# MobilePerceptionLab/EventCalib

Measured on NVIDIA B200. Metric: events/sec (detection+residual eval), higher is better.
Workload: dtype int32 pixels / f64 fit + f64 residuals

## Files before the change

eventcalib_b200/csrc/ecb_api.cu:

```cuda
#include <sched.h>
#include <math.h>
#include <stdarg.h>
#include <stdio.h>
#include <string.h>

#include <algorithm>

#include "ecb_window.cuh"

int ecb_fail(ecb_ctx *ctx, int code, const char *fmt, ...) {
    char buf[512];
    va_list ap;
    va_start(ap, fmt);
    vsnprintf(buf, sizeof buf, fmt, ap);
    va_end(ap);
    if (ctx) ctx->err = buf;
    return code;
}

int ecb_check(ecb_ctx *ctx, cudaError_t e, const char *what) {
    if (e == cudaSuccess) return ECB_OK;
    return ecb_fail(ctx, ECB_ERR_CUDA, "CUDA error %s: %s", what, cudaGetErrorString(e));
}

// ... 102 lines not shown
        cudaGetLastError();
        return 0;
    }
    return n;
}

int ecb_ctx_create(int device, void *stream, ecb_ctx **out) {
    if (!out) return ECB_ERR_ARG;
    *out = nullptr;
    int count = 0;
    if (cudaGetDeviceCount(&count) != cudaSuccess || count <= 0 || device < 0 || device >= count) return ECB_ERR_CUDA;
    if (cudaSetDevice(device) != cudaSuccess) return ECB_ERR_CUDA;
    ecb_ctx *c = new ecb_ctx();
    c->device = device;
    cudaDeviceProp prop;
    if (cudaGetDeviceProperties(&prop, device) != cudaSuccess) {
        delete c;
        return ECB_ERR_CUDA;
    }
    c->sm_count = prop.multiProcessorCount;
    c->smem_optin = (int) prop.sharedMemPerBlockOptin;
    if (stream) {
        c->stream = (cudaStream_t) stream;
    } else {
        if (cudaStreamCreateWithFlags(&c->stream, cudaStreamNonBlocking) != cudaSuccess) {
            delete c;
            return ECB_ERR_CUDA;
        }
        c->own_stream = true;
    }
    if (const char *e = getenv("ECB_BLOCKING_SYNC"))
        if (atoi(e) > 0 && cudaEventCreateWithFlags(&c->sync_ev, (atoi(e) == 1 ? cudaEventBlockingSync : 0) | cudaEventDisableTiming) == cudaSuccess)
            c->sync_mode = atoi(e) == 1 ? 1 : 2;
    *out = c;
    return ECB_OK;
}

void ecb_cost_free(ecb_ctx *ctx);
void ecb_covariance_free(ecb_ctx *ctx);

void ecb_ctx_destroy(ecb_ctx *c) {
    if (!c) return;
    cudaSetDevice(c->device);
    cudaStreamSynchronize(c->stream);
    ecb_covariance_free(c);
    ecb_cost_free(c);
    DevBuf *bufs[] = {&c->ev_raw, &c->ev_t, &c->ev_xyp, &c->ev_flag, &c->win_t, &c->win_lohi, &c->win_ptoff, &c->summary,
                      &c->arrive, &c->pts[0], &c->pts[1], &c->labels[0], &c->labels[1], &c->scratch, &c->ktab, &c->kmem,
                      &c->cand, &c->status, &c->db_pix, &c->db_off, &c->db_labels, &c->db_hdr, &c->db_scratch, &c->db_dims,
                      &c->fit_in, &c->fit_off, &c->fit_out, &c->db_hdr_b, &c->db_ktab, &c->db_counter, &c->kd_tree, &c->bfs_key,
                      &c->bfs_items, &c->bfs_front, &c->bfs_tab, &c->ord_htab, &c->pair_tab, &c->pose_io};
    for (DevBuf *b : bufs)
        if (b->p) cudaFree(b->p);
    for (DevBuf &b : c->gh)
        if (b.p) cudaFree(b.p);
    for (int i = 0; i < ECB_N_STAGES; ++i)
        for (int j = 0; j < 2; ++j)
            if (c->pev[i][j]) cudaEventDestroy(c->pev[i][j]);
    if (c->sync_ev) cudaEventDestroy(c->sync_ev);
    if (c->pinned) cudaFreeHost(c->pinned);
    if (c->up) cudaFreeHost(c->up);
    if (c->own_stream) cudaStreamDestroy(c->stream);
    delete c;
}

const char *ecb_last_error(const ecb_ctx *ctx) { return ctx ? ctx->err.c_str() : "null context"; }
// ... 655 lines not shown
```

eventcalib_b200/csrc/ecb_common.cuh:

```cuda
#pragma once
#include <cuda_runtime.h>
#include <stdint.h>

#include <string>
#include <vector>

#include "../../include/eventcalib_b200.h"

#define ECB_MAX_EPS 15
#define ECB_NONE 0xFFFFFFFFu
#define ECB_GH_MAXD 4
#define ECB_GH_NBUF 32

#define ECB_PIX_X(p) ((p) & 0x7FFFu)
#define ECB_PIX_Y(p) (((p) >> 15) & 0x7FFFu)
#define ECB_PIX_POL(p) ((p) >> 31)
#define ECB_PIX_XY(p) ((p) & 0x3FFFFFFFu)
#define ECB_PIX_INVALID 0x40000000u

struct DevBuf {
    void *p = nullptr;
    size_t cap = 0;
};

struct ecb_ctx {
    int device = 0;
    cudaStream_t stream = nullptr;
    bool own_stream = false;
    std::string err;
    uint64_t launches = 0;
    int sm_count = 148;
    int smem_optin = 0;
    int width = 0, height = 0;
    bool prof = false;
    int sync_mode = 0;
    cudaEvent_t sync_ev = nullptr;
    cudaEvent_t pev[ECB_N_STAGES][2] = {};
    bool pev_used[ECB_N_STAGES] = {};

    int64_t n_events = 0;
    DevBuf ev_raw, ev_t, ev_xyp, ev_flag;
    int n_win = 0;
    ecb_frontend_params fp{};
    DevBuf win_t, win_lohi, win_ptoff, summary, arrive, pts[2], labels[2], scratch, ktab, kmem, cand, status, pair_tab;
    int max_k_auto = 128;
    std::vector<int64_t> h_lohi, h_ptoff;
    int64_t total_points = 0;
    int cand_stride = 0;
    DevBuf kd_tree, bfs_key, bfs_items, bfs_front, bfs_tab;
    DevBuf ord_htab;
    int ord_htab_n = 0;
    DevBuf db_pix, db_off, db_labels, db_hdr, db_scratch, db_dims, db_hdr_b, db_ktab, db_counter;
    DevBuf gh[ECB_GH_NBUF];
    DevBuf fit_in, fit_off, fit_out;
    void *pinned = nullptr;
    size_t pinned_cap = 0;
    void *up = nullptr;
    size_t up_cap = 0, up_off = 0;
    void *cost = nullptr;
    void *cov = nullptr;
    uint64_t spline_gen = 0;
    uint32_t const_intrinsics = 0;
    DevBuf pose_io;
    uint64_t events_gen = 0;
};

struct EcbSplineView {
    const double *knots;
// ... 40 lines not shown
__device__ __forceinline__ uint32_t warp_incl_scan(uint32_t v) {
    const unsigned lane = threadIdx.x & 31;
#pragma unroll
    for (int o = 1; o < 32; o <<= 1) {
        uint32_t t = __shfl_up_sync(0xffffffffu, v, o);
        if (lane >= (unsigned) o) v += t;
    }
    return v;
}

__device__ __forceinline__ uint32_t block_excl_scan(uint32_t v, uint32_t *ws, uint32_t *total) {
    const unsigned lane = threadIdx.x & 31, wid = threadIdx.x >> 5, nw = (blockDim.x + 31) >> 5;
    uint32_t inc = warp_incl_scan(v);
    __syncthreads();
    if (lane == 31) ws[wid] = inc;
    __syncthreads();
    if (wid == 0) {
        uint32_t w = lane < nw ? ws[lane] : 0;
        uint32_t wi = warp_incl_scan(w);
        ws[lane] = wi - w;
        if (lane == 31) ws[32] = wi;
    }
    __syncthreads();
    *total = ws[32];
    return ws[wid] + inc - v;
}

__device__ __forceinline__ uint32_t row_bits(const uint32_t *row, int x0, int len) {
    const int wi = x0 >> 5, sh = x0 & 31;
    uint64_t v = (uint64_t) row[wi] | ((uint64_t) row[wi + 1] << 32);
    return (uint32_t) (v >> sh) & (len >= 32 ? 0xFFFFFFFFu : ((1u << len) - 1u));
}
__device__ __forceinline__ uint32_t test_bit(const uint32_t *row, int x) { return (row[x >> 5] >> (x & 31)) & 1u; }
#endif
```

eventcalib_b200/csrc/ecb_cost.cu:

```cuda
#include <stdlib.h>
#include <string.h>

#include <algorithm>
#include <cmath>
#include <vector>

#include "ecb_bspline.cuh"
#include "ecb_camera.h"
#include "ecb_common.cuh"
#include "ecb_residual_so3.h"

namespace {

constexpr int NE_THREADS = 256;
constexpr int NE_WARPS = NE_THREADS / 32;
constexpr int TILE_ROWS = 34, TILE_LD = 36;
constexpr int N_TILES = 10;
constexpr int PART_E32 = N_TILES * 64, PART_E33 = PART_E32 + 32, PART_SC = PART_E33 + 32, PART_STRIDE = PART_SC + 8;
constexpr int CHUNK = 2048;
constexpr int OUT_STRIDE = 33 * 33 + 33;

struct CostState {
    int n_splines = 0, total_cp = 0, total_spans = 0;
    std::vector<int> n_cp, cp_off, span_off, knot_off;
    std::vector<double> knots;
    double radius = 1.75, huber = 0.35;
    bool use_circ = false;
    int so3 = 0;
    int64_t n_res = 0;
    int n_items = 0;
    DevBuf d_knots, d_knot_off, d_ncp, d_cp_off, d_span_off;
    DevBuf obs, lm, tt, spl, basis, cp0, span;
    DevBuf span_start, items, part, out, params, cost_part, flags;
    DevBuf ev_flag, ev_cnt, ev_tag, kf_t, kf_circ, kf_c32, lm_tab, sel_event, sel_circle;
    std::vector<int64_t> h_span_start;
    bool assoc = false;
    int assoc_K = 0, assoc_n_circ = 0;
    uint64_t assoc_events_gen = 0;
    const double *assoc_kf_t = nullptr;
    double assoc_gate2 = 0.0;
    DevBuf rep_r, rep_key[2], rep_idx[2], rep_hist, rep_start, rep_out, rep_kf;
    DevBuf rep_io;
    DevBuf rej[9];
    uint64_t xch_last_epoch = 0;
    uint32_t xch_generation = 0;
};

CostState *state(ecb_ctx *ctx) {
    if (!ctx->cost) ctx->cost = new CostState();
    return (CostState *) ctx->cost;
}

__global__ void k_prepare(const double *__restrict__ t, const int *__restrict__ spl, int64_t n, const double *__restrict__ knots,
                          const int *__restrict__ knot_off, const int *__restrict__ ncp, const int *__restrict__ cp_off,
                          const int *__restrict__ span_off, double *__restrict__ basis, int *__restrict__ cp0,
                          int *__restrict__ span, uint32_t *__restrict__ flags) {
    const int64_t k = (int64_t) blockIdx.x * blockDim.x + threadIdx.x;
    if (k >= n) return;
    const int s = spl[k];
    const double *kn = knots + knot_off[s];
    const int nk = ncp[s] + 4;
    const double u = t[k];
    if (!(u >= kn[0] && u <= kn[nk - 1])) {
        atomicOr(flags, 1u);
        span[k] = 0;
        cp0[k] = 0;
        return;
// ... 17 lines not shown
    int64_t lo = 0, hi = n;
    while (lo < hi) {
        int64_t m = (lo + hi) >> 1;
        if (span[m] < s) lo = m + 1; else hi = m;
    }
    start[s] = lo;
}

struct Item {
    int64_t begin, end;
    int span, pad;
};

struct NeArgs {
    const double *obs, *lm, *basis;
    const int *circ;
    const double *lm_tab;
    const int *cp0;
    const Item *items;
    int n_items;
    const double *params;
    int total_cp;
    double radius, huber;
    double *part;
    const int *go;
};

__device__ __forceinline__ void dmma(double &c0, double &c1, double a, double b) {
    asm volatile("mma.sync.aligned.m8n8k4.row.col.f64.f64.f64.f64 {%0,%1}, {%2}, {%3}, {%0,%1};\n"
                 : "+d"(c0), "+d"(c1)
                 : "d"(a), "d"(b));
}

template <int MINB, bool SO3>
__global__ void __launch_bounds__(NE_THREADS, MINB) k_normal_eq(const NeArgs a) {
    extern __shared__ __align__(16) double sm_tiles[];
    if (a.go && *a.go == 0) return;
    const int lane = threadIdx.x & 31, wid = threadIdx.x >> 5;
    double *tile = sm_tiles + (size_t) wid * TILE_ROWS * TILE_LD;
    const int g = lane >> 2, t = lane & 3;
    const double *intr = a.params, *rot = a.params + 9, *trans = a.params + 9 + 4 * (size_t) a.total_cp;
    const int gw = blockIdx.x * NE_WARPS + wid, nw = gridDim.x * NE_WARPS;
    for (int it = gw; it < a.n_items; it += nw) {
        const Item item = a.items[it];
        double acc[N_TILES][2];
#pragma unroll
        for (int i = 0; i < N_TILES; ++i) acc[i][0] = acc[i][1] = 0.0;
        double e32 = 0.0, e33 = 0.0;
        double s3232 = 0.0, s3233 = 0.0, s3333 = 0.0, cost = 0.0;
        for (int64_t base = item.begin; base < item.end; base += 32) {
            const int64_t k = base + lane;
            double res = 0.0;
            __syncwarp();
            if (k < item.end) {
                const int c0 = a.cp0[k];
                const double4 b4 = reinterpret_cast<const double4 *>(a.basis)[k];
                const double b[4] = {b4.x, b4.y, b4.z, b4.w};
                const double2 o = reinterpret_cast<const double2 *>(a.obs)[k];
                const double *L = a.circ ? a.lm_tab + 3 * a.circ[k] : a.lm + 3 * k;
                const double Lx = L[0], Ly = L[1], Lz = L[2];
                const EcbResidualOut r =
                    SO3 ? ecb_residual_so3<true, TILE_LD>(intr, rot + 4 * (size_t) c0, trans + 3 * (size_t) c0, b, o.x, o.y,
                                                          Lx, Ly, Lz, a.radius, a.huber,
                                                          tile + lane)
                        : ecb_residual<true, TILE_LD>(intr, rot + 4 * (size_t) c0, trans + 3 * (size_t) c0, b, o.x, o.y,
                                                      Lx, Ly, Lz, a.radius, a.huber,
                                                      tile + lane);
                res = r.res;
                cost += r.cost;
            } else {
#pragma unroll
                for (int c = 0; c < 33; ++c) tile[c * TILE_LD + lane] = 0.0;
            }
            tile[33 * TILE_LD + lane] = res;
            __syncwarp();
            {
                const double x32 = tile[32 * TILE_LD + lane];
                s3232 += x32 * x32;
                s3233 += x32 * res;
                s3333 += res * res;
            }
#pragma unroll
            for (int ks = 0; ks < 8; ++ks) {
                double f[4];
#pragma unroll
                for (int G = 0; G < 4; ++G) f[G] = tile[(8 * G + g) * TILE_LD + 4 * ks + t];
                int ti = 0;
#pragma unroll
                for (int I = 0; I < 4; ++I)
#pragma unroll
                    for (int Jt = I; Jt < 4; ++Jt) {
                        dmma(acc[ti][0], acc[ti][1], f[I], f[Jt]);
                        ++ti;
                    }
#pragma unroll
                for (int q = 0; q < 4; ++q) {
                    const int kk = (4 * ks + q + (lane >> 2)) & 31;
                    const double aj = tile[lane * TILE_LD + kk];
                    e32 += aj * tile[32 * TILE_LD + kk];
                    e33 += aj * tile[33 * TILE_LD + kk];
                }
            }
        }
        double *p = a.part + (size_t) it * PART_STRIDE;
#pragma unroll
        for (int ti = 0; ti < N_TILES; ++ti) reinterpret_cast<double2 *>(p + ti * 64)[lane] = make_double2(acc[ti][0], acc[ti][1]);
        p[PART_E32 + lane] = e32;
        p[PART_E33 + lane] = e33;
#pragma unroll
        for (int o = 16; o > 0; o >>= 1) {
            cost += __shfl_xor_sync(0xffffffffu, cost, o);
            s3232 += __shfl_xor_sync(0xffffffffu, s3232, o);
            s3233 += __shfl_xor_sync(0xffffffffu, s3233, o);
            s3333 += __shfl_xor_sync(0xffffffffu, s3333, o);
        }
        if (lane == 0) {
            p[PART_SC + 0] = s3232;
            p[PART_SC + 1] = s3233;
            p[PART_SC + 2] = s3333;
            p[PART_SC + 3] = cost;
        }
    }
}

__global__ void k_reduce_spans(const double *__restrict__ part, const int *__restrict__ item_start, int n_spans,
                               double *__restrict__ out, const int *__restrict__ go = nullptr) {
    const int s = blockIdx.x;
    if (s >= n_spans || (go && *go == 0)) return;
    const int i0 = item_start[s], i1 = item_start[s + 1];
    double *o = out + (size_t) s * OUT_STRIDE;
    for (int e = threadIdx.x; e < PART_SC + 2; e += blockDim.x) {
        double v = 0.0;
        for (int it = i0; it < i1; ++it) v += part[(size_t) it * PART_STRIDE + e];
        if (e < PART_E32) {
            const int ti = e >> 6, r = (e >> 3) & 7, c = e & 7;
            int I = 0, rem = ti;
            while (rem >= 4 - I) {
                rem -= 4 - I;
                ++I;
            }
            const int Jt = I + rem;
            const int i = 8 * I + r, j = 8 * Jt + c;
            if (I != Jt || i <= j) {
                o[i * 33 + j] = v;
                o[j * 33 + i] = v;
            }
        } else if (e < PART_E33) {
            const int j = e - PART_E32;
            o[32 * 33 + j] = v;
            o[j * 33 + 32] = v;
        } else if (e < PART_SC) {
            o[1089 + (e - PART_E33)] = v;
        } else if (e == PART_SC) {
// ... 177 lines not shown
    const double *intr = params, *rot = params + 9, *trans = params + 9 + 4 * (size_t) total_cp;
    double c = 0.0;
    for (int64_t k = (int64_t) blockIdx.x * 256 + threadIdx.x; k < n; k += (int64_t) gridDim.x * 256) {
        const int c0 = cp0[k];
        const double4 b4 = reinterpret_cast<const double4 *>(basis)[k];
        const double b[4] = {b4.x, b4.y, b4.z, b4.w};
        const double2 o = reinterpret_cast<const double2 *>(obs)[k];
        const double *L = circ ? lm_tab + 3 * circ[k] : lm + 3 * k;
        const double Lx = L[0], Ly = L[1], Lz = L[2];
        c += SO3 ? ecb_residual_so3<false>(intr, rot + 4 * (size_t) c0, trans + 3 * (size_t) c0, b, o.x, o.y, Lx, Ly, Lz, radius,
                                           huber, nullptr).cost
                 : ecb_residual<false>(intr, rot + 4 * (size_t) c0, trans + 3 * (size_t) c0, b, o.x, o.y, Lx, Ly, Lz, radius, huber,
                                       nullptr).cost;
    }
    sh[threadIdx.x] = c;
    __syncthreads();
    for (int o = 128; o > 0; o >>= 1) {
        if (threadIdx.x < o) sh[threadIdx.x] += sh[threadIdx.x + o];
        __syncthreads();
    }
    if (threadIdx.x == 0) block_part[blockIdx.x] = sh[0];
}

struct AssocArgs {
    const double *ev_t;
    const uint32_t *ev_xyp;
    int64_t n_ev;
    const double *knots;
    const int *knot_off, *ncp;
    int n_splines;
    const double *kf_t, *kf_circ, *lm_tab;
    const float2 *kf_c32;
    int K, n_circ, n_circ32;
    double gate2;
    const int *cp_off, *span_off;
    double *basis;
    int *cp0, *span;
};

__device__ __forceinline__ int segment_of(const AssocArgs &a, double u) {
    for (int q = 0; q < a.n_splines; ++q) {
        const double *kn = a.knots + a.knot_off[q];
        if (u >= kn[0] && u <= kn[a.ncp[q] + 3]) return q;
    }
    return -1;
}

__device__ __forceinline__ int assoc_one(const AssocArgs &a, int64_t i, int *spline_out) {
    const double u = a.ev_t[i];
    const int s = segment_of(a, u);
    if (s < 0) return -1;
    *spline_out = s;
    int lo = 0, hi = a.K;
    while (lo < hi) {
        const int m = (lo + hi) >> 1;
        if (a.kf_t[m] < u) lo = m + 1; else hi = m;
    }
    int best = lo < a.K ? lo : a.K - 1;
    if (lo > 0 && (lo >= a.K || (u - a.kf_t[lo - 1]) <= (a.kf_t[lo] - u))) best = lo - 1;
    const double dt = u - a.kf_t[best];
    if (!(__dmul_rn(dt, dt) < a.gate2)) return -1;
    const uint32_t e = a.ev_xyp[i];
    if (e & ECB_PIX_INVALID) return -1;
    const double x = (double) ECB_PIX_X(e), y = (double) ECB_PIX_Y(e);
    const double *c = a.kf_circ + (size_t) best * a.n_circ * 3;
    int bi = -1;
    double bd = 0.0;
    {
        const float xf = (float) ECB_PIX_X(e), yf = (float) ECB_PIX_Y(e);
        const float4 *c4 = reinterpret_cast<const float4 *>(a.kf_c32 + (size_t) best * a.n_circ32);
        uint32_t k1 = 0xFFFFFFFFu, k2 = 0xFFFFFFFFu;
#pragma unroll 6
        for (int q = 0; q < a.n_circ32; q += 2) {
            const float4 cc = c4[q >> 1];
            const float dx0 = xf - cc.x, dy0 = yf - cc.y, dx1 = xf - cc.z, dy1 = yf - cc.w;
            const uint32_t ka = (__float_as_uint(fmaf(dx0, dx0, dy0 * dy0)) & 0xFFFFFF00u) | (uint32_t) q;
            const uint32_t kb = (__float_as_uint(fmaf(dx1, dx1, dy1 * dy1)) & 0xFFFFFF00u) | (uint32_t) (q + 1);
            k2 = min(k2, max(ka, k1));
            k1 = min(k1, ka);
            k2 = min(k2, max(kb, k1));
            k1 = min(k1, kb);
        }
        const float d1 = __uint_as_float(k1 & 0xFFFFFF00u), d2 = __uint_as_float(k2 | 0xFFu);
        if (d2 > d1 * 1.0001f + 0.02f) {
            bi = (int) (k1 & 0xFFu);
            if (bi >= a.n_circ || c[3 * bi + 2] < 0) return -1;
            const double dx = x - c[3 * bi], dy = y - c[3 * bi + 1];
            bd = __dadd_rn(__dmul_rn(dx, dx), __dmul_rn(dy, dy));
        } else {
            for (int q = 0; q < a.n_circ; ++q) {
                if (c[3 * q + 2] < 0) continue;
                const double dx = x - c[3 * q], dy = y - c[3 * q + 1];
                const double dd = __dadd_rn(__dmul_rn(dx, dx), __dmul_rn(dy, dy));
                if (bi < 0 || dd < bd) {
                    bi = q;
                    bd = dd;
                }
            }
        }
    }
    if (bi < 0) return -1;
    if (!(fabs(sqrt(bd) - c[3 * bi + 2]) < 5.0)) return -1;
    return bi;
}

constexpr int AS_THREADS = 256;

__global__ void k_circ32(const double *__restrict__ c, int K, int n_circ, int n_circ32, float2 *__restrict__ o) {
    const int i = blockIdx.x * blockDim.x + threadIdx.x;
    if (i >= K * n_circ32) return;
    const int k = i / n_circ32, q = i - k * n_circ32;
    float2 v = make_float2(3e18f, 3e18f);
    if (q < n_circ) {
        const double *p = c + ((size_t) k * n_circ + q) * 3;
        if (!(p[2] < 0)) v = make_float2((float) p[0], (float) p[1]);
    }
    o[i] = v;
}

__device__ __forceinline__ int nearest_kf(const double *kf_t, int K, double u) {
    int lo = 0, hi = K;
    while (lo < hi) {
        const int m = (lo + hi) >> 1;
        if (kf_t[m] < u) lo = m + 1; else hi = m;
    }
    int best = lo < K ? lo : K - 1;
    if (lo > 0 && (lo >= K || (u - kf_t[lo - 1]) <= (kf_t[lo] - u))) best = lo - 1;
    return best;
}

__global__ void __launch_bounds__(AS_THREADS) k_assoc_count(const AssocArgs a, uint16_t *__restrict__ tag,
                                                           uint32_t *__restrict__ block_cnt) {
    __shared__ uint32_t ws[33];
    const int64_t i = (int64_t) blockIdx.x * AS_THREADS + threadIdx.x;
    int s = 0;
    const int bi = i < a.n_ev ? assoc_one(a, i, &s) : -1;
    if (i < a.n_ev) tag[i] = bi >= 0 ? (uint16_t) ((s << 8) | (bi + 1)) : (uint16_t) 0;
    uint32_t tot;
    block_excl_scan(bi >= 0 ? 1u : 0u, ws, &tot);
    if (threadIdx.x == 0) block_cnt[blockIdx.x] = tot;
}

__global__ void k_scan_blocks(uint32_t *cnt, int n, int64_t *off, int64_t *total) {
    __shared__ uint32_t ws[33];
    const int per = (n + (int) blockDim.x - 1) / (int) blockDim.x;
    const int b = min(n, (int) threadIdx.x * per), e = min(n, b + per);
    uint32_t sum = 0;
    for (int i = b; i < e; ++i) sum += cnt[i];
    uint32_t tot;
    int64_t run = block_excl_scan(sum, ws, &tot);
    for (int i = b; i < e; ++i) {
        off[i] = run;
        run += cnt[i];
    }
    if (threadIdx.x == 0) *total = tot;
}

__global__ void __launch_bounds__(AS_THREADS) k_assoc_write(const AssocArgs a, const uint16_t *__restrict__ tag,
                                                           const int64_t *__restrict__ block_off,
                                                           double *__restrict__ obs, double *__restrict__ lm,
                                                           double *__restrict__ tt, int *__restrict__ spl,
                                                           int64_t *__restrict__ sel_event, int *__restrict__ sel_circle) {
    __shared__ uint32_t ws[33];
    const int64_t i = (int64_t) blockIdx.x * AS_THREADS + threadIdx.x;
    const uint32_t tg = i < a.n_ev ? tag[i] : 0u;
    uint32_t tot;
    const uint32_t ex = block_excl_scan(tg ? 1u : 0u, ws, &tot);
    if (tg) {
        const int bi = (int) (tg & 0xFF) - 1, s = (int) (tg >> 8);
// ... 712 lines not shown
    int rc;
    const int64_t n = ctx->n_events;
    const int nb = (int) ((n + AS_THREADS - 1) / AS_THREADS);
    if (!on_device) {
        if ((rc = ecb_reserve(ctx, st->kf_t, (size_t) n_keyframes * 8))) return rc;
        if ((rc = ecb_reserve(ctx, st->kf_circ, (size_t) n_keyframes * n_circles * 24))) return rc;
    }
    if ((rc = ecb_reserve(ctx, st->lm_tab, (size_t) n_circles * 24))) return rc;
    const int n_circ32 = (n_circles + 1) & ~1;
    if ((rc = ecb_reserve(ctx, st->kf_c32, (size_t) n_keyframes * n_circ32 * 8))) return rc;
    if (n_circles > 254 || st->n_splines > 255) return ecb_fail(ctx, ECB_ERR_UNSUPPORTED, "more than 254 circles or 255 spline segments");
    if ((rc = ecb_reserve(ctx, st->ev_cnt, (size_t) nb * 4 + 16))) return rc;
    if ((rc = ecb_reserve(ctx, st->ev_tag, (size_t) n * 2 + 16))) return rc;
    if ((rc = ecb_reserve(ctx, st->ev_flag, (size_t) nb * 8 + 16))) return rc;
    const double *d_kf_t = kf_time, *d_kf_circ = kf_circles;
    if (!on_device) {
        if ((rc = ecb_h2d(ctx, st->kf_t.p, kf_time, (size_t) n_keyframes * 8))) return rc;
        if ((rc = ecb_h2d(ctx, st->kf_circ.p, kf_circles, (size_t) n_keyframes * n_circles * 24))) return rc;
        if ((rc = ecb_h2d(ctx, st->lm_tab.p, landmarks_xyz, (size_t) n_circles * 24))) return rc;
        d_kf_t = (const double *) st->kf_t.p;
        d_kf_circ = (const double *) st->kf_circ.p;
    } else {
        ECB_CUDA(ctx, cudaMemcpyAsync(st->lm_tab.p, landmarks_xyz, (size_t) n_circles * 24, cudaMemcpyDeviceToDevice, ctx->stream));
    }
    AssocArgs a;
    assoc_args(ctx, st, a);
    a.kf_t = d_kf_t;
    a.kf_circ = d_kf_circ;
    a.kf_c32 = (const float2 *) st->kf_c32.p;
    a.K = n_keyframes;
    a.n_circ = n_circles;
    a.n_circ32 = n_circ32;
    a.gate2 = 5 * motion_time_step * 5 * motion_time_step;
    ECB_PROF_BEGIN(ctx, ECB_STAGE_ASSOC);
    k_circ32<<<(n_keyframes * n_circ32 + 255) / 256, 256, 0, ctx->stream>>>(d_kf_circ, n_keyframes, n_circles,
                                                                           n_circ32, (float2 *) st->kf_c32.p);
    ECB_LAUNCHED(ctx);
    k_assoc_count<<<nb, AS_THREADS, 0, ctx->stream>>>(a, (uint16_t *) st->ev_tag.p, (uint32_t *) st->ev_cnt.p);
    ECB_LAUNCHED(ctx);
    int64_t *d_total = (int64_t *) st->ev_flag.p + nb;
    k_scan_blocks<<<1, 1024, 0, ctx->stream>>>((uint32_t *) st->ev_cnt.p, nb, (int64_t *) st->ev_flag.p, d_total);
    ECB_LAUNCHED(ctx);
    int64_t total = 0;
    if ((rc = ecb_d2h(ctx, &total, d_total, 8))) return rc;
    bool fused = true;
    {
        std::vector<std::pair<double, double>> rg;
        size_t ko2 = 0;
        for (int q = 0; q < st->n_splines; ++q) {
            rg.emplace_back(st->knots[ko2], st->knots[ko2 + (size_t) st->n_cp[(size_t) q] + 3]);
            ko2 += (size_t) st->n_cp[(size_t) q] + 4;
        }
        std::sort(rg.begin(), rg.end());
        for (size_t q = 1; q < rg.size(); ++q)
            if (!(rg[q].first > rg[q - 1].second))
                return ecb_fail(ctx, ECB_ERR_UNSUPPORTED,
                                "spline knot ranges overlap ([%g, %g] and [%g, %g]): an event inside both would need one residual "
                                "per spline", rg[q - 1].first, rg[q - 1].second, rg[q].first, rg[q].second);
        size_t ko = 0;
        double prev_end = -1e300;
        for (int q = 0; q < st->n_splines; ++q) {
            const double b = st->knots[ko], e = st->knots[ko + (size_t) st->n_cp[(size_t) q] + 3];
            if (!(b > prev_end)) fused = false;
            prev_end = e;
            ko += (size_t) st->n_cp[(size_t) q] + 4;
        }
    }
    if ((rc = write_assoc_records(ctx, st, a, nb, total, fused))) return rc;
    ECB_PROF_END(ctx, ECB_STAGE_ASSOC);
    if ((rc = ecb_check(ctx, cudaGetLastError(), "association kernels"))) return rc;
    st->n_res = total;
// ... 24 lines not shown

static long long exchange_timeout_clocks(ecb_ctx *ctx) {
    static const double secs = getenv("ECB_EXCHANGE_TIMEOUT_S") ? atof(getenv("ECB_EXCHANGE_TIMEOUT_S")) : 30.0;
    static int khz_of[64] = {0};
    const int d = ctx->device & 63;
    if (khz_of[d] == 0) {
        int khz = 1965000;
        cudaDeviceGetAttribute(&khz, cudaDevAttrClockRate, ctx->device);
        khz_of[d] = khz > 0 ? khz : 1965000;
    }
    return (long long) (secs * 1e3 * (double) khz_of[d]);
}

static void fill_ne_args(CostState *st, NeArgs &a, const double *d_params, const int *d_go) {
    a.obs = (const double *) st->obs.p;
    a.lm = (const double *) st->lm.p;
    a.circ = st->use_circ ? (const int *) st->sel_circle.p : nullptr;
    a.lm_tab = (const double *) st->lm_tab.p;
    a.basis = (const double *) st->basis.p;
    a.cp0 = (const int *) st->cp0.p;
    a.items = (const Item *) st->items.p;
    a.n_items = st->n_items;
    a.params = d_params;
    a.total_cp = st->total_cp;
    a.radius = st->radius;
    a.huber = st->huber;
    a.part = (double *) st->part.p;
    a.go = d_go;
}

static int launch_normal_eq_kernel(ecb_ctx *ctx, CostState *st, const double *d_params, const int *d_go) {
    NeArgs a;
    fill_ne_args(st, a, d_params, d_go);
    const size_t smem = (size_t) NE_WARPS * TILE_ROWS * TILE_LD * 8;
    static const int variant = getenv("ECB_NE_VARIANT") ? atoi(getenv("ECB_NE_VARIANT")) : 2;
    void (*kern)(const NeArgs) = st->so3 ? k_normal_eq<1, true> : (variant == 1 ? k_normal_eq<1, false> : k_normal_eq<2, false>);
    ECB_CUDA(ctx, cudaFuncSetAttribute(kern, cudaFuncAttributeMaxDynamicSharedMemorySize, (int) smem));
    const int grid = std::min((st->n_items + NE_WARPS - 1) / NE_WARPS, ctx->sm_count * ((variant == 1 || st->so3) ? 1 : 2));
    kern<<<grid, NE_THREADS, smem, ctx->stream>>>(a);
    ECB_LAUNCHED(ctx);
    return ECB_OK;
}

static const int *item_start_of(CostState *st) {
    return (const int *) ((const char *) st->items.p + (size_t) std::max(st->n_items, 1) * sizeof(Item));
}

static void span_range(CostState *st, int &lo, int &hi) {
    lo = 0;
    hi = -1;
    for (int s = 0; s < st->total_spans; ++s)
        if (st->h_span_start[(size_t) s + 1] > st->h_span_start[(size_t) s]) {
            if (hi < 0) lo = s;
            hi = s;
        }
}

int ecb_cost_dev_eval(ecb_ctx *ctx, const double *d_params, const int *d_go, double *d_cost) {
    CostState *st = (CostState *) ctx->cost;
    int rc;
    if ((rc = ecb_reserve(ctx, st->cost_part, 4096 * 8))) return rc;
    if (st->n_res == 0) {
        ECB_CUDA(ctx, cudaMemsetAsync(d_cost, 0, 8, ctx->stream));
        return ECB_OK;
    }
    const int grid = (int) std::min<int64_t>((st->n_res + 255) / 256, (int64_t) ctx->sm_count * 8);
// ... 619 lines not shown
```

eventcalib_b200/csrc/ecb_window.cu:

```cuda
#include "ecb_cluster.cuh"
#include "ecb_window.cuh"

namespace {

constexpr int ING_REC = 256;
constexpr int ING_BYTES = ING_REC * 25;
constexpr int ING_THREADS = 256;

__device__ __forceinline__ uint32_t ld_unaligned32(const uint32_t *w, int byte_off) {
    const int wi = byte_off >> 2, sh = (byte_off & 3) * 8;
    return __funnelshift_r(w[wi], w[wi + 1], sh);
}

constexpr int ING_STAGES = 4;

__device__ __forceinline__ uint32_t smem_u32(const void *p) { return (uint32_t) __cvta_generic_to_shared(p); }
__device__ __forceinline__ void mbar_init(uint64_t *bar, int count) {
    asm volatile("mbarrier.init.shared::cta.b64 [%0], %1;" ::"r"(smem_u32(bar)), "r"(count));
}
__device__ __forceinline__ void mbar_expect_tx(uint64_t *bar, uint32_t bytes) {
    asm volatile("mbarrier.arrive.expect_tx.shared::cta.b64 _, [%0], %1;" ::"r"(smem_u32(bar)), "r"(bytes) : "memory");
}
__device__ __forceinline__ void mbar_wait(uint64_t *bar, uint32_t parity) {
    asm volatile(
        "{\n"
        ".reg .pred p;\n"
        "WAIT_%=:\n"
        "mbarrier.try_wait.parity.shared::cta.b64 p, [%0], %1;\n"
        "@p bra DONE_%=;\n"
        "bra WAIT_%=;\n"
        "DONE_%=:\n"
        "}" ::"r"(smem_u32(bar)), "r"(parity) : "memory");
}
__device__ __forceinline__ void bulk_g2s(void *dst, const void *src, uint32_t bytes, uint64_t *bar) {
    asm volatile("cp.async.bulk.shared::cluster.global.mbarrier::complete_tx::bytes [%0], [%1], %2, [%3];" ::"r"(smem_u32(dst)),
                 "l"(src), "r"(bytes), "r"(smem_u32(bar))
                 : "memory");
}

__global__ void __launch_bounds__(ING_THREADS) k_ingest(const uint8_t *__restrict__ raw, int64_t n, int W, int H,
                                                         double *__restrict__ out_t, uint32_t *__restrict__ out_xyp,
                                                         uint32_t *__restrict__ flags) {
    __shared__ __align__(128) uint32_t sm[ING_STAGES][ING_BYTES / 4 + 4];
    __shared__ __align__(8) uint64_t full[ING_STAGES];
    const int64_t n_tiles = (n + ING_REC - 1) / ING_REC;
    const int64_t total_bytes = n * 25;
    const int tid = threadIdx.x;
    const int64_t my_tiles = n_tiles > blockIdx.x ? (n_tiles - blockIdx.x + gridDim.x - 1) / gridDim.x : 0;
    auto issue = [&](int64_t it) {
        const int st = (int) (it % ING_STAGES);
        const int64_t byte0 = (blockIdx.x + it * gridDim.x) * (int64_t) ING_BYTES;
        const uint32_t bytes = (uint32_t) (min((int64_t) ING_BYTES, total_bytes - byte0) & ~(int64_t) 15);
        mbar_expect_tx(&full[st], bytes);
        if (bytes) bulk_g2s(sm[st], raw + byte0, bytes, &full[st]);
    };
    if (tid == 0) {
        for (int st = 0; st < ING_STAGES; ++st) mbar_init(&full[st], 1);
        asm volatile("fence.mbarrier_init.release.cluster;" ::: "memory");
    }
    __syncthreads();
    if (tid == 0)
        for (int64_t it = 0; it < my_tiles && it < ING_STAGES; ++it) issue(it);
    uint32_t bad = 0;
    for (int64_t it = 0; it < my_tiles; ++it) {
        const int st = (int) (it % ING_STAGES);
// ... 239 lines not shown
```

Measured before the change: 2.619 billion.

## Add per-keyframe spatial cell candidate lists for event-circle association

Builds a per-keyframe grid of 16x16 pixel cells, each holding up to 7 candidate circles that could be nearest to any pixel in the cell. The association kernel then checks only those candidates and falls back to the full scan when a cell overflows or the nearest two are too close to call. The aim is to replace the full scan over all circles per event with a few lookups. It costs an extra precompute kernel with a shared array of fixed size (254 circles), and it adds a risk of results differing when the candidate bounds are near ties.

```diff
diff --git a/eventcalib_b200/csrc/ecb_api.cu b/eventcalib_b200/csrc/ecb_api.cu
--- a/eventcalib_b200/csrc/ecb_api.cu
+++ b/eventcalib_b200/csrc/ecb_api.cu
@@ -158,6 +158,7 @@
     if (const char *e = getenv("ECB_BLOCKING_SYNC"))
         if (atoi(e) > 0 && cudaEventCreateWithFlags(&c->sync_ev, (atoi(e) == 1 ? cudaEventBlockingSync : 0) | cudaEventDisableTiming) == cudaSuccess)
             c->sync_mode = atoi(e) == 1 ? 1 : 2;
+    if (const char *e = getenv("ECB_ASSOC_SCAN")) c->assoc_scan = atoi(e) == 1;
     *out = c;
     return ECB_OK;
 }
diff --git a/eventcalib_b200/csrc/ecb_common.cuh b/eventcalib_b200/csrc/ecb_common.cuh
--- a/eventcalib_b200/csrc/ecb_common.cuh
+++ b/eventcalib_b200/csrc/ecb_common.cuh
@@ -34,6 +34,7 @@
     int width = 0, height = 0;
     bool prof = false;
     int sync_mode = 0;
+    bool assoc_scan = false;
     cudaEvent_t sync_ev = nullptr;
     cudaEvent_t pev[ECB_N_STAGES][2] = {};
     bool pev_used[ECB_N_STAGES] = {};
diff --git a/eventcalib_b200/csrc/ecb_cost.cu b/eventcalib_b200/csrc/ecb_cost.cu
--- a/eventcalib_b200/csrc/ecb_cost.cu
+++ b/eventcalib_b200/csrc/ecb_cost.cu
@@ -32,7 +32,7 @@
     DevBuf d_knots, d_knot_off, d_ncp, d_cp_off, d_span_off;
     DevBuf obs, lm, tt, spl, basis, cp0, span;
     DevBuf span_start, items, part, out, params, cost_part, flags;
-    DevBuf ev_flag, ev_cnt, ev_tag, kf_t, kf_circ, kf_c32, lm_tab, sel_event, sel_circle;
+    DevBuf ev_flag, ev_cnt, ev_tag, kf_t, kf_circ, kf_c32, kf_cells, lm_tab, sel_event, sel_circle;
     std::vector<int64_t> h_span_start;
     bool assoc = false;
     int assoc_K = 0, assoc_n_circ = 0;
@@ -446,6 +446,8 @@
     const double *kf_t, *kf_circ, *lm_tab;
     const float2 *kf_c32;
     int K, n_circ, n_circ32;
+    const uint2 *cells;
+    int cell_nx, cell_ny;
     double gate2;
     const int *cp_off, *span_off;
     double *basis;
@@ -460,26 +462,22 @@
     return -1;
 }
 
-__device__ __forceinline__ int assoc_one(const AssocArgs &a, int64_t i, int *spline_out) {
-    const double u = a.ev_t[i];
-    const int s = segment_of(a, u);
-    if (s < 0) return -1;
-    *spline_out = s;
-    int lo = 0, hi = a.K;
+__device__ __forceinline__ int nearest_kf(const double *kf_t, int K, double u) {
+    int lo = 0, hi = K;
     while (lo < hi) {
         const int m = (lo + hi) >> 1;
-        if (a.kf_t[m] < u) lo = m + 1; else hi = m;
-    }
-    int best = lo < a.K ? lo : a.K - 1;
-    if (lo > 0 && (lo >= a.K || (u - a.kf_t[lo - 1]) <= (a.kf_t[lo] - u))) best = lo - 1;
-    const double dt = u - a.kf_t[best];
-    if (!(__dmul_rn(dt, dt) < a.gate2)) return -1;
-    const uint32_t e = a.ev_xyp[i];
-    if (e & ECB_PIX_INVALID) return -1;
+        if (kf_t[m] < u) lo = m + 1; else hi = m;
+    }
+    int best = lo < K ? lo : K - 1;
+    if (lo > 0 && (lo >= K || (u - kf_t[lo - 1]) <= (kf_t[lo] - u))) best = lo - 1;
+    return best;
+}
+
+__device__ __forceinline__ int nearest_circle_scan(const AssocArgs &a, int best, uint32_t e, double &bd) {
     const double x = (double) ECB_PIX_X(e), y = (double) ECB_PIX_Y(e);
     const double *c = a.kf_circ + (size_t) best * a.n_circ * 3;
     int bi = -1;
-    double bd = 0.0;
+    bd = 0.0;
     {
         const float xf = (float) ECB_PIX_X(e), yf = (float) ECB_PIX_Y(e);
         const float4 *c4 = reinterpret_cast<const float4 *>(a.kf_c32 + (size_t) best * a.n_circ32);
@@ -513,42 +511,125 @@
             }
         }
     }
+    return bi;
+}
+
+constexpr int AC_CELL = 16;
+constexpr int AC_CAP = 7;
+constexpr int AC_FULL = 0xFF;
+constexpr int AC_THREADS = 256;
+
+__global__ void __launch_bounds__(AC_THREADS) k_assoc_cells(const double *__restrict__ kf_circ, int n_circ, int n_circ32,
+                                                            int nx, int ny, float2 *__restrict__ c32, uint2 *__restrict__ cells) {
+    __shared__ double sc[3 * 254];
+    const int k = blockIdx.x;
+    const double *c = kf_circ + (size_t) k * n_circ * 3;
+    int bad = 0;
+    for (int q = threadIdx.x; q < n_circ32; q += AC_THREADS) {
+        float2 v = make_float2(3e18f, 3e18f);
+        if (q < n_circ) {
+            const double x = c[3 * q], y = c[3 * q + 1], r = c[3 * q + 2];
+            sc[3 * q] = x;
+            sc[3 * q + 1] = y;
+            sc[3 * q + 2] = r;
+            if (!(r < 0)) {
+                v = make_float2((float) x, (float) y);
+                bad |= !(fabs(x) < INFINITY && fabs(y) < INFINITY);
+            }
+        }
+        c32[(size_t) k * n_circ32 + q] = v;
+    }
+    bad = __syncthreads_or(bad);
+    if (!cells) return;
+    const int ncell = nx * ny;
+    for (int cell = threadIdx.x; cell < ncell; cell += AC_THREADS) {
+        const int gy = cell / nx, gx = cell - gy * nx;
+        const double x0 = gx * AC_CELL, x1 = x0 + (AC_CELL - 1), y0 = gy * AC_CELL, y1 = y0 + (AC_CELL - 1);
+        double D = INFINITY;
+        for (int q = 0; q < n_circ; ++q) {
+            if (sc[3 * q + 2] < 0) continue;
+            const double cx = sc[3 * q], cy = sc[3 * q + 1];
+            const double ex = fmax(fabs(x0 - cx), fabs(x1 - cx)), ey = fmax(fabs(y0 - cy), fabs(y1 - cy));
+            D = fmin(D, __dadd_rn(__dmul_rn(ex, ex), __dmul_rn(ey, ey)));
+        }
+        const double B = __dadd_rn(__dmul_rn(D, 1.0 + 1e-9), 1e-9);
+        uint64_t list = 0;
+        int n = 0;
+        for (int q = 0; q < n_circ; ++q) {
+            if (sc[3 * q + 2] < 0) continue;
+            const double cx = sc[3 * q], cy = sc[3 * q + 1];
+            const double ex = cx < x0 ? x0 - cx : (cx > x1 ? cx - x1 : 0.0), ey = cy < y0 ? y0 - cy : (cy > y1 ? cy - y1 : 0.0);
+            if (__dadd_rn(__dmul_rn(ex, ex), __dmul_rn(ey, ey)) <= B) {
+                if (n < AC_CAP) list |= (uint64_t) q << (8 * (n + 1));
+                ++n;
+            }
+        }
+        list |= (uint64_t) (bad || n > AC_CAP ? AC_FULL : n);
+        cells[(size_t) k * ncell + cell] = make_uint2((uint32_t) list, (uint32_t) (list >> 32));
+    }
+}
+
+__device__ __forceinline__ int nearest_circle_cells(const AssocArgs &a, int best, uint32_t e, double &bd) {
+    const uint32_t px = ECB_PIX_X(e), py = ECB_PIX_Y(e);
+    const uint32_t gx = px / AC_CELL, gy = py / AC_CELL;
+    if (gx < (uint32_t) a.cell_nx && gy < (uint32_t) a.cell_ny) {
+        const uint2 rec = a.cells[((size_t) best * a.cell_ny + gy) * a.cell_nx + gx];
+        const int n = (int) (rec.x & 0xFFu);
+        if (n == 0) return -1;
+        if (n != AC_FULL) {
+            const float xf = (float) px, yf = (float) py;
+            const float2 *c2 = a.kf_c32 + (size_t) best * a.n_circ32;
+            uint64_t list = ((uint64_t) rec.y << 32 | rec.x) >> 8;
+            uint32_t k1 = 0xFFFFFFFFu, k2 = 0x7F000000u;
+#pragma unroll 1
+            for (int j = 0; j < n; ++j, list >>= 8) {
+                const uint32_t q = (uint32_t) list & 0xFFu;
+                const float2 cc = c2[q];
+                const float dx = xf - cc.x, dy = yf - cc.y;
+                const uint32_t kq = (__float_as_uint(fmaf(dx, dx, dy * dy)) & 0xFFFFFF00u) | q;
+                k2 = min(k2, max(kq, k1));
+                k1 = min(k1, kq);
+            }
+            const float d1 = __uint_as_float(k1 & 0xFFFFFF00u), d2 = __uint_as_float(k2 | 0xFFu);
+            if (d2 > d1 * 1.0001f + 0.02f) {
+                const int bi = (int) (k1 & 0xFFu);
+                const double *c = a.kf_circ + ((size_t) best * a.n_circ + bi) * 3;
+                const double dx = (double) px - c[0], dy = (double) py - c[1];
+                bd = __dadd_rn(__dmul_rn(dx, dx), __dmul_rn(dy, dy));
+                return bi;
+            }
+        }
+    }
+    return nearest_circle_scan(a, best, e, bd);
+}
+
+template <bool CELLS>
+__device__ __forceinline__ int assoc_one(const AssocArgs &a, int64_t i, int *spline_out) {
+    const double u = a.ev_t[i];
+    const int s = segment_of(a, u);
+    if (s < 0) return -1;
+    *spline_out = s;
+    const int best = nearest_kf(a.kf_t, a.K, u);
+    const double dt = u - a.kf_t[best];
+    if (!(__dmul_rn(dt, dt) < a.gate2)) return -1;
+    const uint32_t e = a.ev_xyp[i];
+    if (e & ECB_PIX_INVALID) return -1;
+    double bd;
+    const int bi = CELLS ? nearest_circle_cells(a, best, e, bd) : nearest_circle_scan(a, best, e, bd);
     if (bi < 0) return -1;
-    if (!(fabs(sqrt(bd) - c[3 * bi + 2]) < 5.0)) return -1;
+    if (!(fabs(sqrt(bd) - a.kf_circ[((size_t) best * a.n_circ + bi) * 3 + 2]) < 5.0)) return -1;
     return bi;
 }
 
 constexpr int AS_THREADS = 256;
 
-__global__ void k_circ32(const double *__restrict__ c, int K, int n_circ, int n_circ32, float2 *__restrict__ o) {
-    const int i = blockIdx.x * blockDim.x + threadIdx.x;
-    if (i >= K * n_circ32) return;
-    const int k = i / n_circ32, q = i - k * n_circ32;
-    float2 v = make_float2(3e18f, 3e18f);
-    if (q < n_circ) {
-        const double *p = c + ((size_t) k * n_circ + q) * 3;
-        if (!(p[2] < 0)) v = make_float2((float) p[0], (float) p[1]);
-    }
-    o[i] = v;
-}
-
-__device__ __forceinline__ int nearest_kf(const double *kf_t, int K, double u) {
-    int lo = 0, hi = K;
-    while (lo < hi) {
-        const int m = (lo + hi) >> 1;
-        if (kf_t[m] < u) lo = m + 1; else hi = m;
-    }
-    int best = lo < K ? lo : K - 1;
-    if (lo > 0 && (lo >= K || (u - kf_t[lo - 1]) <= (kf_t[lo] - u))) best = lo - 1;
-    return best;
-}
-
+template <bool CELLS>
 __global__ void __launch_bounds__(AS_THREADS) k_assoc_count(const AssocArgs a, uint16_t *__restrict__ tag,
                                                            uint32_t *__restrict__ block_cnt) {
     __shared__ uint32_t ws[33];
     const int64_t i = (int64_t) blockIdx.x * AS_THREADS + threadIdx.x;
     int s = 0;
-    const int bi = i < a.n_ev ? assoc_one(a, i, &s) : -1;
+    const int bi = i < a.n_ev ? assoc_one<CELLS>(a, i, &s) : -1;
     if (i < a.n_ev) tag[i] = bi >= 0 ? (uint16_t) ((s << 8) | (bi + 1)) : (uint16_t) 0;
     uint32_t tot;
     block_excl_scan(bi >= 0 ? 1u : 0u, ws, &tot);
@@ -1327,11 +1408,20 @@
     a.n_circ = n_circles;
     a.n_circ32 = n_circ32;
     a.gate2 = 5 * motion_time_step * 5 * motion_time_step;
+    a.cell_nx = (ctx->width + AC_CELL - 1) / AC_CELL;
+    a.cell_ny = (ctx->height + AC_CELL - 1) / AC_CELL;
+    const int64_t n_lists = (int64_t) n_keyframes * a.cell_nx * a.cell_ny;
+    const bool cells = !ctx->assoc_scan && n_lists > 0 && n_lists <= n;
+    if (cells) {
+        if ((rc = ecb_reserve(ctx, st->kf_cells, (size_t) n_lists * sizeof(uint2)))) return rc;
+        a.cells = (const uint2 *) st->kf_cells.p;
+    }
     ECB_PROF_BEGIN(ctx, ECB_STAGE_ASSOC);
-    k_circ32<<<(n_keyframes * n_circ32 + 255) / 256, 256, 0, ctx->stream>>>(d_kf_circ, n_keyframes, n_circles,
-                                                                           n_circ32, (float2 *) st->kf_c32.p);
+    k_assoc_cells<<<n_keyframes, AC_THREADS, 0, ctx->stream>>>(d_kf_circ, n_circles, n_circ32, a.cell_nx, a.cell_ny,
+                                                               (float2 *) st->kf_c32.p, cells ? (uint2 *) st->kf_cells.p : nullptr);
     ECB_LAUNCHED(ctx);
-    k_assoc_count<<<nb, AS_THREADS, 0, ctx->stream>>>(a, (uint16_t *) st->ev_tag.p, (uint32_t *) st->ev_cnt.p);
+    (cells ? k_assoc_count<true> : k_assoc_count<false>)<<<nb, AS_THREADS, 0, ctx->stream>>>(a, (uint16_t *) st->ev_tag.p,
+                                                                                             (uint32_t *) st->ev_cnt.p);
     ECB_LAUNCHED(ctx);
     int64_t *d_total = (int64_t *) st->ev_flag.p + nb;
     k_scan_blocks<<<1, 1024, 0, ctx->stream>>>((uint32_t *) st->ev_cnt.p, nb, (int64_t *) st->ev_flag.p, d_total);
```

Result: no change. 2.626 billion (median of 6 runs) (+0.3%).

## Warp-specialize normal-equation kernel with producer residual warps and mbarrier ring

Applied to the files above, without the earlier changes.

Adds a warp-specialized normal-equation kernel and makes it the default. Producer warps compute residuals and Jacobian columns into a per-consumer ring of shared-memory tiles. Consumer warps run the f64 MMA Gram accumulation, and mbarrier full/empty handshakes connect the two sides. The goal is to overlap the latency-bound residual evaluation with the tensor-core Gram products instead of serialising them within one warp. In exchange it runs one block per SM, adds barrier overhead, and changes how occupancy and shared memory are spent; the old path is still available through an env var.

```diff
diff --git a/eventcalib_b200/csrc/ecb_common.cuh b/eventcalib_b200/csrc/ecb_common.cuh
--- a/eventcalib_b200/csrc/ecb_common.cuh
+++ b/eventcalib_b200/csrc/ecb_common.cuh
@@ -140,4 +140,23 @@
     return (uint32_t) (v >> sh) & (len >= 32 ? 0xFFFFFFFFu : ((1u << len) - 1u));
 }
 __device__ __forceinline__ uint32_t test_bit(const uint32_t *row, int x) { return (row[x >> 5] >> (x & 31)) & 1u; }
+
+__device__ __forceinline__ uint32_t smem_u32(const void *p) { return (uint32_t) __cvta_generic_to_shared(p); }
+__device__ __forceinline__ void mbar_init(uint64_t *bar, int count) {
+    asm volatile("mbarrier.init.shared::cta.b64 [%0], %1;" ::"r"(smem_u32(bar)), "r"(count));
+}
+__device__ __forceinline__ void mbar_arrive(uint64_t *bar) {
+    asm volatile("mbarrier.arrive.shared::cta.b64 _, [%0];" ::"r"(smem_u32(bar)) : "memory");
+}
+__device__ __forceinline__ void mbar_wait(uint64_t *bar, uint32_t parity) {
+    asm volatile(
+        "{\n"
+        ".reg .pred p;\n"
+        "WAIT_%=:\n"
+        "mbarrier.try_wait.parity.shared::cta.b64 p, [%0], %1;\n"
+        "@p bra DONE_%=;\n"
+        "bra WAIT_%=;\n"
+        "DONE_%=:\n"
+        "}" ::"r"(smem_u32(bar)), "r"(parity) : "memory");
+}
 #endif
diff --git a/eventcalib_b200/csrc/ecb_cost.cu b/eventcalib_b200/csrc/ecb_cost.cu
--- a/eventcalib_b200/csrc/ecb_cost.cu
+++ b/eventcalib_b200/csrc/ecb_cost.cu
@@ -116,14 +116,86 @@
                  : "d"(a), "d"(b));
 }
 
+struct NeRecord {
+    int c0;
+    double b[4];
+    double ox, oy, Lx, Ly, Lz;
+};
+
+__device__ __forceinline__ NeRecord ne_load(const NeArgs &a, int64_t k) {
+    NeRecord r;
+    r.c0 = a.cp0[k];
+    const double4 b4 = reinterpret_cast<const double4 *>(a.basis)[k];
+    r.b[0] = b4.x, r.b[1] = b4.y, r.b[2] = b4.z, r.b[3] = b4.w;
+    const double2 o = reinterpret_cast<const double2 *>(a.obs)[k];
+    r.ox = o.x, r.oy = o.y;
+    const double *L = a.circ ? a.lm_tab + 3 * a.circ[k] : a.lm + 3 * k;
+    r.Lx = L[0], r.Ly = L[1], r.Lz = L[2];
+    return r;
+}
+
+template <bool SO3>
+__device__ __forceinline__ EcbResidualOut ne_residual(const NeArgs &a, const NeRecord &r, double *col) {
+    const double *intr = a.params, *rot = a.params + 9, *trans = a.params + 9 + 4 * (size_t) a.total_cp;
+    return SO3 ? ecb_residual_so3<true, TILE_LD>(intr, rot + 4 * (size_t) r.c0, trans + 3 * (size_t) r.c0, r.b, r.ox, r.oy,
+                                                 r.Lx, r.Ly, r.Lz, a.radius, a.huber, col)
+               : ecb_residual<true, TILE_LD>(intr, rot + 4 * (size_t) r.c0, trans + 3 * (size_t) r.c0, r.b, r.ox, r.oy,
+                                             r.Lx, r.Ly, r.Lz, a.radius, a.huber, col);
+}
+
+__device__ __forceinline__ void ne_gram_group(const double *tile, int lane, double (&acc)[N_TILES][2], double &e32, double &e33) {
+    const int g = lane >> 2, t = lane & 3;
+#pragma unroll
+    for (int ks = 0; ks < 8; ++ks) {
+        double f[4];
+#pragma unroll
+        for (int G = 0; G < 4; ++G) f[G] = tile[(8 * G + g) * TILE_LD + 4 * ks + t];
+        int ti = 0;
+#pragma unroll
+        for (int I = 0; I < 4; ++I)
+#pragma unroll
+            for (int Jt = I; Jt < 4; ++Jt) {
+                dmma(acc[ti][0], acc[ti][1], f[I], f[Jt]);
+                ++ti;
+            }
+#pragma unroll
+        for (int q = 0; q < 4; ++q) {
+            const int kk = (4 * ks + q + (lane >> 2)) & 31;
+            const double aj = tile[lane * TILE_LD + kk];
+            e32 += aj * tile[32 * TILE_LD + kk];
+            e33 += aj * tile[33 * TILE_LD + kk];
+        }
+    }
+}
+
+__device__ __forceinline__ void ne_write_part(const NeArgs &a, int it, int lane, const double (&acc)[N_TILES][2], double e32,
+                                              double e33, double s3232, double s3233, double s3333, double cost) {
+    double *p = a.part + (size_t) it * PART_STRIDE;
+#pragma unroll
+    for (int ti = 0; ti < N_TILES; ++ti) reinterpret_cast<double2 *>(p + ti * 64)[lane] = make_double2(acc[ti][0], acc[ti][1]);
+    p[PART_E32 + lane] = e32;
+    p[PART_E33 + lane] = e33;
+#pragma unroll
+    for (int o = 16; o > 0; o >>= 1) {
+        cost += __shfl_xor_sync(0xffffffffu, cost, o);
+        s3232 += __shfl_xor_sync(0xffffffffu, s3232, o);
+        s3233 += __shfl_xor_sync(0xffffffffu, s3233, o);
+        s3333 += __shfl_xor_sync(0xffffffffu, s3333, o);
+    }
+    if (lane == 0) {
+        p[PART_SC + 0] = s3232;
+        p[PART_SC + 1] = s3233;
+        p[PART_SC + 2] = s3333;
+        p[PART_SC + 3] = cost;
+    }
+}
+
 template <int MINB, bool SO3>
 __global__ void __launch_bounds__(NE_THREADS, MINB) k_normal_eq(const NeArgs a) {
     extern __shared__ __align__(16) double sm_tiles[];
     if (a.go && *a.go == 0) return;
     const int lane = threadIdx.x & 31, wid = threadIdx.x >> 5;
     double *tile = sm_tiles + (size_t) wid * TILE_ROWS * TILE_LD;
-    const int g = lane >> 2, t = lane & 3;
-    const double *intr = a.params, *rot = a.params + 9, *trans = a.params + 9 + 4 * (size_t) a.total_cp;
     const int gw = blockIdx.x * NE_WARPS + wid, nw = gridDim.x * NE_WARPS;
     for (int it = gw; it < a.n_items; it += nw) {
         const Item item = a.items[it];
@@ -137,19 +209,7 @@
             double res = 0.0;
             __syncwarp();
             if (k < item.end) {
-                const int c0 = a.cp0[k];
-                const double4 b4 = reinterpret_cast<const double4 *>(a.basis)[k];
-                const double b[4] = {b4.x, b4.y, b4.z, b4.w};
-                const double2 o = reinterpret_cast<const double2 *>(a.obs)[k];
-                const double *L = a.circ ? a.lm_tab + 3 * a.circ[k] : a.lm + 3 * k;
-                const double Lx = L[0], Ly = L[1], Lz = L[2];
-                const EcbResidualOut r =
-                    SO3 ? ecb_residual_so3<true, TILE_LD>(intr, rot + 4 * (size_t) c0, trans + 3 * (size_t) c0, b, o.x, o.y,
-                                                          Lx, Ly, Lz, a.radius, a.huber,
-                                                          tile + lane)
-                        : ecb_residual<true, TILE_LD>(intr, rot + 4 * (size_t) c0, trans + 3 * (size_t) c0, b, o.x, o.y,
-                                                      Lx, Ly, Lz, a.radius, a.huber,
-                                                      tile + lane);
+                const EcbResidualOut r = ne_residual<SO3>(a, ne_load(a, k), tile + lane);
                 res = r.res;
                 cost += r.cost;
             } else {
@@ -164,45 +224,77 @@
                 s3233 += x32 * res;
                 s3333 += res * res;
             }
+            ne_gram_group(tile, lane, acc, e32, e33);
+        }
+        ne_write_part(a, it, lane, acc, e32, e33, s3232, s3233, s3333, cost);
+    }
+}
+
+constexpr int NE_CONS = 4;
+__device__ __forceinline__ int ne_cost_slot(int lane) { return (lane >> 2) * TILE_LD + 32 + (lane & 3); }
+
+template <bool SO3, int NP, int R>
+__global__ void __launch_bounds__(32 * (NE_CONS + NP), 1) k_normal_eq_pipe(const NeArgs a) {
+    constexpr int PPC = NP / NE_CONS, TILE = TILE_ROWS * TILE_LD;
+    static_assert(NP % NE_CONS == 0 && R >= PPC, "ring sizing");
+    extern __shared__ __align__(16) double sm_tiles[];
+    __shared__ uint64_t full[NE_CONS * R], empty[NE_CONS * R];
+    if (a.go && *a.go == 0) return;
+    const int lane = threadIdx.x & 31, wid = threadIdx.x >> 5, c = wid % NE_CONS;
+    if (threadIdx.x < NE_CONS * R) {
+        mbar_init(&full[threadIdx.x], 32);
+        mbar_init(&empty[threadIdx.x], 32);
+    }
+    __syncthreads();
+    double *ring = sm_tiles + (size_t) c * R * TILE;
+    uint64_t *fb = full + c * R, *eb = empty + c * R;
+    const int nc = gridDim.x * NE_CONS;
+    int j = 0;
+    if (wid < NE_CONS) {
+        for (int it = blockIdx.x * NE_CONS + c; it < a.n_items; it += nc) {
+            const Item item = a.items[it];
+            double acc[N_TILES][2];
 #pragma unroll
-            for (int ks = 0; ks < 8; ++ks) {
-                double f[4];
+            for (int i = 0; i < N_TILES; ++i) acc[i][0] = acc[i][1] = 0.0;
+            double e32 = 0.0, e33 = 0.0;
+            double s3232 = 0.0, s3233 = 0.0, s3333 = 0.0, cost = 0.0;
+            for (int64_t base = item.begin; base < item.end; base += 32, ++j) {
+                const double *tile = ring + (j % R) * TILE;
+                mbar_wait(fb + j % R, (j / R) & 1);
+                __syncwarp();
+                if (base + lane < item.end) cost += tile[ne_cost_slot(lane)];
+                {
+                    const double x32 = tile[32 * TILE_LD + lane], res = tile[33 * TILE_LD + lane];
+                    s3232 += x32 * x32;
+                    s3233 += x32 * res;
+                    s3333 += res * res;
+                }
+                ne_gram_group(tile, lane, acc, e32, e33);
+                mbar_arrive(eb + j % R);
+            }
+            ne_write_part(a, it, lane, acc, e32, e33, s3232, s3233, s3333, cost);
+        }
+    } else {
+        const int q = wid / NE_CONS - 1;
+        for (int it = blockIdx.x * NE_CONS + c; it < a.n_items; it += nc) {
+            const Item item = a.items[it];
+            for (int64_t base = item.begin; base < item.end; base += 32, ++j) {
+                if (j % PPC != q) continue;
+                const int64_t k = base + lane;
+                double *tile = ring + (j % R) * TILE;
+                if (k < item.end) {
+                    const NeRecord rec = ne_load(a, k);
+                    mbar_wait(eb + j % R, ((j / R) & 1) ^ 1);
+                    const EcbResidualOut r = ne_residual<SO3>(a, rec, tile + lane);
+                    tile[33 * TILE_LD + lane] = r.res;
+                    tile[ne_cost_slot(lane)] = r.cost;
+                } else {
+                    mbar_wait(eb + j % R, ((j / R) & 1) ^ 1);
 #pragma unroll
-                for (int G = 0; G < 4; ++G) f[G] = tile[(8 * G + g) * TILE_LD + 4 * ks + t];
-                int ti = 0;
-#pragma unroll
-                for (int I = 0; I < 4; ++I)
-#pragma unroll
-                    for (int Jt = I; Jt < 4; ++Jt) {
-                        dmma(acc[ti][0], acc[ti][1], f[I], f[Jt]);
-                        ++ti;
-                    }
-#pragma unroll
-                for (int q = 0; q < 4; ++q) {
-                    const int kk = (4 * ks + q + (lane >> 2)) & 31;
-                    const double aj = tile[lane * TILE_LD + kk];
-                    e32 += aj * tile[32 * TILE_LD + kk];
-                    e33 += aj * tile[33 * TILE_LD + kk];
+                    for (int r = 0; r < 34; ++r) tile[r * TILE_LD + lane] = 0.0;
                 }
+                mbar_arrive(fb + j % R);
             }
-        }
-        double *p = a.part + (size_t) it * PART_STRIDE;
-#pragma unroll
-        for (int ti = 0; ti < N_TILES; ++ti) reinterpret_cast<double2 *>(p + ti * 64)[lane] = make_double2(acc[ti][0], acc[ti][1]);
-        p[PART_E32 + lane] = e32;
-        p[PART_E33 + lane] = e33;
-#pragma unroll
-        for (int o = 16; o > 0; o >>= 1) {
-            cost += __shfl_xor_sync(0xffffffffu, cost, o);
-            s3232 += __shfl_xor_sync(0xffffffffu, s3232, o);
-            s3233 += __shfl_xor_sync(0xffffffffu, s3233, o);
-            s3333 += __shfl_xor_sync(0xffffffffu, s3333, o);
-        }
-        if (lane == 0) {
-            p[PART_SC + 0] = s3232;
-            p[PART_SC + 1] = s3233;
-            p[PART_SC + 2] = s3333;
-            p[PART_SC + 3] = cost;
         }
     }
 }
@@ -1422,6 +1514,18 @@
 static int launch_normal_eq_kernel(ecb_ctx *ctx, CostState *st, const double *d_params, const int *d_go) {
     NeArgs a;
     fill_ne_args(st, a, d_params, d_go);
+    static const int pipe = getenv("ECB_NE_PIPE") ? atoi(getenv("ECB_NE_PIPE")) : 1;
+    if (pipe) {
+        constexpr int NP = 12, R = 4, NP_SO3 = 4, R_SO3 = 3;
+        void (*kern)(const NeArgs) = st->so3 ? k_normal_eq_pipe<true, NP_SO3, R_SO3> : k_normal_eq_pipe<false, NP, R>;
+        const int threads = 32 * (NE_CONS + (st->so3 ? NP_SO3 : NP));
+        const size_t smem = (size_t) NE_CONS * (st->so3 ? R_SO3 : R) * TILE_ROWS * TILE_LD * 8;
+        ECB_CUDA(ctx, cudaFuncSetAttribute(kern, cudaFuncAttributeMaxDynamicSharedMemorySize, (int) smem));
+        const int grid = std::min((st->n_items + NE_CONS - 1) / NE_CONS, ctx->sm_count);
+        kern<<<grid, threads, smem, ctx->stream>>>(a);
+        ECB_LAUNCHED(ctx);
+        return ECB_OK;
+    }
     const size_t smem = (size_t) NE_WARPS * TILE_ROWS * TILE_LD * 8;
     static const int variant = getenv("ECB_NE_VARIANT") ? atoi(getenv("ECB_NE_VARIANT")) : 2;
     void (*kern)(const NeArgs) = st->so3 ? k_normal_eq<1, true> : (variant == 1 ? k_normal_eq<1, false> : k_normal_eq<2, false>);
diff --git a/eventcalib_b200/csrc/ecb_window.cu b/eventcalib_b200/csrc/ecb_window.cu
--- a/eventcalib_b200/csrc/ecb_window.cu
+++ b/eventcalib_b200/csrc/ecb_window.cu
@@ -14,23 +14,8 @@
 
 constexpr int ING_STAGES = 4;
 
-__device__ __forceinline__ uint32_t smem_u32(const void *p) { return (uint32_t) __cvta_generic_to_shared(p); }
-__device__ __forceinline__ void mbar_init(uint64_t *bar, int count) {
-    asm volatile("mbarrier.init.shared::cta.b64 [%0], %1;" ::"r"(smem_u32(bar)), "r"(count));
-}
 __device__ __forceinline__ void mbar_expect_tx(uint64_t *bar, uint32_t bytes) {
     asm volatile("mbarrier.arrive.expect_tx.shared::cta.b64 _, [%0], %1;" ::"r"(smem_u32(bar)), "r"(bytes) : "memory");
-}
-__device__ __forceinline__ void mbar_wait(uint64_t *bar, uint32_t parity) {
-    asm volatile(
-        "{\n"
-        ".reg .pred p;\n"
-        "WAIT_%=:\n"
-        "mbarrier.try_wait.parity.shared::cta.b64 p, [%0], %1;\n"
-        "@p bra DONE_%=;\n"
-        "bra WAIT_%=;\n"
-        "DONE_%=:\n"
-        "}" ::"r"(smem_u32(bar)), "r"(parity) : "memory");
 }
 __device__ __forceinline__ void bulk_g2s(void *dst, const void *src, uint32_t bytes, uint64_t *bar) {
     asm volatile("cp.async.bulk.shared::cluster.global.mbarrier::complete_tx::bytes [%0], [%1], %2, [%3];" ::"r"(smem_u32(dst)),
```

New measurement: 2.631 billion before, 2.687 billion after (median of 6 runs). 1.02x the previous value.
